# fema-ffrd/gpras

Hardware: AMD Instinct MI355X
Metric: gp_fits_per_sec (higher is better)
Workload: dtype f64; 1 GPU; BASELINE configs[1] as the many-independent-cells workload: exact GP N=4096 d=8 RBF, fit F1 = kernel build + blocked fp64-MFMA Cholesky + alpha + LML, per cell; cells = y columns of one training set with per-cell hyperparameters (the reference's per-mode models); n_train=4096, d=8, kernel=RBF, collective=none (one process), launcher=single process

## Files before the change

gpras_amd/_lib.py:

```python

from __future__ import annotations

import ctypes as C
from pathlib import Path

import numpy as np

import os

LIB_PATH = Path(os.environ["GPRX_LIBRARY"]) if os.environ.get("GPRX_LIBRARY") else Path(__file__).resolve().parent / "libgprx.so"

GPRX_OK, GPRX_EINVAL, GPRX_ENOTPD, GPRX_EHIP, GPRX_ENOMEM, GPRX_ESTATE, GPRX_ERCCL = range(7)
UNIQUE_ID_BYTES = 128
TRAIN_VARIANCE, TRAIN_LENGTHSCALE, TRAIN_NOISE, TRAIN_Z = 1, 2, 4, 8
GEMM_C_LOWER, GEMM_A_LOWER, GEMM_A_UPPER, GEMM_B_LOWER, GEMM_B_UPPER = 1, 2, 4, 8, 16

DISTANCE_FORMS = {"difference": 0, "expanded": 1}
KERNEL_IDS = {"RBF": 0, "Matern12": 1, "Matern32": 2, "Matern52": 3, "Exponential": 4}


class GprxLibraryError(RuntimeError):
    """libgprx.so is missing or unusable."""


# ... 78 lines not shown
    "gprx_ps_destroy": (C.c_int, [_vp]),
    "gprx_ps_last_error": (C.c_char_p, [_vp]),
    "gprx_ps_set_weights": (C.c_int, [_vp, _vp]),
    "gprx_ps_fit_centerline": (C.c_int, [_vp, _vp, _vp, _vp, _vp, _vp, _i64, _vp]),
    "gprx_ps_timings": (C.c_int, [_vp, _dp]),
    "gprx_ps_rating": (C.c_int, [_vp, _vp, _vp, _i64, _vp, _vp]),
    "gprx_ps_set_boundaries": (C.c_int, [_vp, _vp, _vp, _i64]),
    "gprx_ps_centerline": (C.c_int, [_vp, _vp]),
    "gprx_ps_gather": (C.c_int, [_vp, _vp, _i64, _vp]),
    "gprx_ps_surface": (C.c_int, [_vp, _vp, _vp]),
    "gprx_ps_surface_dev": (C.c_int, [_vp, _i64, _i64, _vp, _i64, _vp, _i64]),
    "gprx_ps_synchronize": (C.c_int, [_vp]),
    "gprx_pca_slab_rows": (C.c_int, [_vp, C.POINTER(_i64)]),
    "gprx_metrics": (C.c_int, [C.c_int, _vp, _vp, _vp, _i64, _i64, C.c_int, C.c_double, _vp, _vp, _vp, C.POINTER(C.c_uint64)]),
    "gprx_metrics_dev": (C.c_int, [C.c_int, _vp, _vp, _vp, _i64, _i64, C.c_int, C.c_double, _vp, _vp, _vp, C.POINTER(C.c_uint64)]),
    "gprx_kmeans_pp": (C.c_int, [C.c_int, _vp, _i64, C.c_int, _vp, C.c_int, C.c_int, _i64, _vp, _vp]),
    "gprx_kmeans_lloyd": (C.c_int, [C.c_int, _vp, _i64, C.c_int, _vp, C.c_int, C.c_double, C.c_int, _vp, _ip, _ip]),
    "gprx_gather_rows": (C.c_int, [C.c_int, _vp, _i64, _i64, _vp, _vp]),
    "gprx_kmat": (C.c_int, [C.c_int, C.c_int, _vp, _i64, _vp, _i64, C.c_int, _vp, C.c_double, C.c_double, _vp, _i64, _i64, _i64, C.c_int]),
    "gprx_gemm": (C.c_int, [C.c_int, C.c_int, C.c_int, _i64, _i64, _i64, C.c_double, _vp, _i64, _vp, _i64, C.c_double, _vp, _i64, C.c_int, C.c_int]),
    "gprx_potrf": (C.c_int, [C.c_int, _vp, _i64, _i64, _i64, _vp, _ip]),
    "gprx_set_tuning": (C.c_int, [C.c_char_p, C.c_int]),
    "gprx_set_handle_tuning": (C.c_int, [_vp, C.c_char_p, C.c_int]),
    "gprx_mfma_f64_peak": (C.c_int, [C.c_int, _dp]),
    "gprx_exp_probe": (C.c_int, [C.c_int, C.c_int, _vp, _i64, _vp]),
}

_lib = None


def load():
    global _lib
    if _lib is not None:
        return _lib
    if not LIB_PATH.exists():
        raise GprxLibraryError(
            f"{LIB_PATH} not found: build it with `python -c 'import __graft_entry__ as g; g.build()'` "
            "(hipcc --offload-arch=gfx950).  gpras_amd has no CPU fallback."
        )
    try:
        lib = C.CDLL(str(LIB_PATH))
    except OSError as exc:
        raise GprxLibraryError(f"cannot load {LIB_PATH}: {exc}") from exc
    for name, (res, args) in PROTOTYPES.items():
        try:
            fn = getattr(lib, name)
# ... 70 lines not shown
```

gpras_amd/csrc/gemm_f64.h:

```cpp
#pragma once
#include <cstdlib>

#include "gprx_common.h"

namespace gprx {

struct GemmArgs {
  const double* A;
  const double* B;
  double* C;
  int64_t lda, ldb, ldc;
  int M, N, K;
  double alpha, beta;
  int flags;
  int tiles_n;
  int tiles_m;
  int nwg;
  int64_t strideA, strideB, strideC;
  int ksplit;
  int64_t slab;
  int inner = 0;
  int64_t cellA = 0, cellB = 0, cellC = 0;
  const double* a_sub = nullptr;
  const double* a_mul = nullptr;
  const double* a_elev = nullptr;
  const double* alpha_tab = nullptr;
  int alpha_stride = 0;
  int persist_slots = 0;
  double* rowsq = nullptr;
  int64_t rowsq_ld = 0;
  int cell_xcd = 0;
};

#ifndef GPRX_GEMM_PFC_DEFAULT
#define GPRX_GEMM_PFC_DEFAULT 1
#endif
#ifndef GPRX_GEMM_DMA_DEFAULT
#define GPRX_GEMM_DMA_DEFAULT 1
#endif
constexpr int GEMM_BK = 16;
constexpr int GEMM_LDK = GEMM_BK;
__device__ __forceinline__ int kc_swz(int row) { return (int)((0xa7a09f5366f7ull >> (3 * (row & 15))) & 7ull); }

template <int BMN>
struct McStride {
  static constexpr int value = BMN + 4;
};

template <int ROWS>
__device__ __forceinline__ void load_kc(d2 (&r)[ROWS / 32], const double* __restrict__ base, int64_t ld, int row0, int nrows_valid,
                                        int k0, int tid) {
#pragma unroll
  for (int i = 0; i < ROWS / 32; ++i) {
    const int q = tid + 256 * i;
    const int row = q >> 3, cc = q & 7;
    if (row0 + row < nrows_valid)
      r[i] = *reinterpret_cast<const d2*>(base + (int64_t)(row0 + row) * ld + k0 + cc * 2);
    else
      r[i] = d2{0.0, 0.0};
  }
}
template <int ROWS>
__device__ __forceinline__ void store_kc(double* s, const d2 (&r)[ROWS / 32], int tid) {
// ... 22 lines not shown
  }
}
template <int COLS>
__device__ __forceinline__ void store_mc(double* s, const d2 (&r)[COLS / 32], int tid) {
#pragma unroll
  for (int i = 0; i < COLS / 32; ++i) {
    const int q = tid + 256 * i;
    const int krow = q / (COLS / 2), cc = q % (COLS / 2);
    *reinterpret_cast<d2*>(s + krow * McStride<COLS>::value + cc * 2) = r[i];
  }
}

__device__ __forceinline__ void glds16(const double* src, double* lds_wave_base) {
  __builtin_amdgcn_global_load_lds((const __attribute__((address_space(1))) void*)src, (__attribute__((address_space(3))) void*)lds_wave_base, 16, 0, 0);
}

template <int TA, int TB, int BM, int BN>
struct GemmSmem {
  static constexpr int A_ELEMS = TA ? GEMM_BK * McStride<BM>::value : BM * GEMM_LDK;
  static constexpr int B_ELEMS = TB ? BN * GEMM_LDK : GEMM_BK * McStride<BN>::value;
  static constexpr int doubles = 2 * (A_ELEMS + B_ELEMS);
};

template <int TA, int TB, int BM, int BN, int PF, int AXF, int DMA>
__device__ __forceinline__ void gemm_tile(GemmArgs p, const int bx_in, const int by_in, const int bz, double* __restrict__ smem) {
  int bx = bx_in, by = by_in;
  if (p.cell_xcd) {
    const int L = bx_in + p.nwg * by_in, slot = L >> 3;
    const int cq = slot / p.nwg;
    by = (L & 7) + 8 * cq;
    bx = slot - cq * p.nwg;
  }
  static_assert(!DMA || (AXF == 0 && (TA == 0 || BM == 64) && (TB == 1 || BN == 64)),
                "the LDS-DMA staging exists for k-contiguous operands and for m/n-contiguous operands of 64-wide tiles");
  constexpr int TM = BM / 32, TN = BN / 32;
  constexpr int A_ELEMS = GemmSmem<TA, TB, BM, BN>::A_ELEMS;
  constexpr int B_ELEMS = GemmSmem<TA, TB, BM, BN>::B_ELEMS;

  const int tid = threadIdx.x;
  const int lane = tid & 63;
  const int wave = tid >> 6;
  const int wm = wave >> 1, wn = wave & 1;
  const int g = lane >> 4, r = lane & 15;

  {
    int entry = by;
    if (p.inner > 0) {
      const int cell = entry / p.inner;
      entry -= cell * p.inner;
      p.A += (int64_t)cell * p.cellA;
      p.B += (int64_t)cell * p.cellB;
      p.C += (int64_t)cell * p.cellC;
      if (p.alpha_tab) p.alpha = p.alpha_tab[(int64_t)cell * p.alpha_stride];
    }
    p.A += (int64_t)entry * p.strideA;
    p.B += (int64_t)entry * p.strideB;
    p.C += (int64_t)entry * p.strideC;
  }
  int bid = bx;
  if (!p.cell_xcd && !(p.flags & (GEMM_A_LOWER | GEMM_A_UPPER | GEMM_B_LOWER | GEMM_B_UPPER))) {
    const int q = p.nwg >> 3, rr = p.nwg & 7, xcd = bid & 7, k = bid >> 3;
    bid = (xcd < rr ? xcd * (q + 1) : rr * (q + 1) + (xcd - rr) * q) + k;
  }
  int ti, tj;
  if (p.flags & GEMM_C_LOWER) {
#ifndef GPRX_BAND
#define GPRX_BAND 4
#endif
    constexpr int R = GPRX_BAND;
    const int tn = p.tiles_n;
    const int tri = tn * (tn + 1) / 2;
    if (bid < tri) {
      int b = (int)((sqrtf((float)(R + 1) * (R + 1) / 4.0f - (float)(R + 1) * R / 2.0f + (float)R * R / 4.0f + 2.0f * (float)bid) -
                     (float)(R + 1) / 2.0f + (float)R / 2.0f) / (float)R);
      if (b < 0) b = 0;
      auto S = [](int bb) { return R * R * bb * (bb - 1) / 2 + bb * R * (R + 1) / 2; };
      while (S(b + 1) <= bid) ++b;
      while (S(b) > bid) --b;
      int u = bid - S(b);
      const int r0 = R * b;
      const int h = (tn - r0 < R) ? tn - r0 : R;
      if (u < h * r0) {
        tj = u / h;
        ti = r0 + u % h;
      } else {
        u -= h * r0;
        int c = 0;
        while (u >= h - c) {
          u -= h - c;
          ++c;
        }
        tj = r0 + c;
        ti = r0 + c + u;
      }
    } else {
      const int rest = bid - tri;
      const int b2 = rest / (R * tn);
      const int u = rest - b2 * R * tn;
      const int left = p.tiles_m - tn - R * b2;
      const int h = left < R ? left : R;
      tj = u / h;
      ti = tn + R * b2 + u % h;
    }
  } else {
    const int tri = p.flags & (GEMM_A_LOWER | GEMM_A_UPPER | GEMM_B_LOWER | GEMM_B_UPPER);
    if (tri == GEMM_B_UPPER || tri == GEMM_B_LOWER) {
      const int cj = bid / p.tiles_m;
      ti = bid % p.tiles_m;
      tj = (tri == GEMM_B_UPPER) ? p.tiles_n - 1 - cj : cj;
    } else if (tri == GEMM_A_LOWER || tri == GEMM_A_UPPER) {
      const int ri = bid / p.tiles_n;
      tj = bid % p.tiles_n;
      ti = (tri == GEMM_A_LOWER) ? p.tiles_m - 1 - ri : ri;
    } else {
      ti = bid / p.tiles_n;
      tj = bid % p.tiles_n;
      if (tri & (GEMM_B_LOWER | GEMM_B_UPPER)) tj = (tj + ti) % p.tiles_n;
    }
  }
  const int m0 = ti * BM, n0 = tj * BN;

  int kbeg = 0, kend = p.K;
  if (p.flags & GEMM_A_LOWER) kend = min(kend, m0 + BM);
  if (p.flags & GEMM_A_UPPER) kbeg = max(kbeg, m0);
  if (p.flags & GEMM_B_LOWER) kbeg = max(kbeg, n0);
  if (p.flags & GEMM_B_UPPER) kend = min(kend, n0 + BN);
// ... 241 lines not shown
#pragma unroll
        for (int q = 0; q < 4; ++q) {
          const int row = m0 + wm * (BM / 2) + a * 16 + g + 4 * q;
          cold[b][q] = (row < p.M && col < p.N) ? p.C[(int64_t)row * p.ldc + col] : 0.0;
        }
      }
    }
#pragma unroll
    for (int b = 0; b < TN; ++b) {
      const int col = n0 + wn * (BN / 2) + b * 16 + r;
#pragma unroll
      for (int q = 0; q < 4; ++q) {
        const int row = m0 + wm * (BM / 2) + a * 16 + g + 4 * q;
        if (row < p.M && col < p.N) {
          double v = alpha * acc[a][b][q];
          if (beta != 0.0) v = __builtin_fma(beta, cold[b][q], v);
          p.C[(int64_t)row * p.ldc + col] = v;
        }
      }
    }
  }
}

template <int TA, int TB, int BM, int BN, int PF = 0, int AXF = 0, int DMA = 0>
__global__ __launch_bounds__(256, (BM * BN >= 128 * 128) ? 2 : (((PF && !DMA) || AXF) ? 3 : 4)) void gemm_f64_kernel(GemmArgs p) {
  __shared__ __attribute__((aligned(16))) double smem[GemmSmem<TA, TB, BM, BN>::doubles];
  gemm_tile<TA, TB, BM, BN, PF, AXF, DMA>(p, (int)blockIdx.x, (int)blockIdx.y, (int)blockIdx.z, smem);
}

template <int BM, int BN, int PF>
__global__ __launch_bounds__(256, (BM * BN >= 128 * 128) ? 2 : 4) void gemm_f64_nt_dma_persistent_kernel(GemmArgs p, int batch) {
  __shared__ __attribute__((aligned(16))) double smem[GemmSmem<0, 1, BM, BN>::doubles];
  const int total = p.nwg * batch;
  for (int t = (int)blockIdx.x; t < total; t += (int)gridDim.x) {
    const int by = t / p.nwg;
    gemm_tile<0, 1, BM, BN, PF, 0, 1>(p, t - by * p.nwg, by, 0, smem);
  }
}

template <int TA, int TB, int BM, int BN>
inline hipError_t launch_gemm_t(hipStream_t st, GemmArgs p, int batch, int nsplit = 1) {
  p.tiles_m = (p.M + BM - 1) / BM;
  p.tiles_n = (p.N + BN - 1) / BN;
  if (p.tiles_m == 0 || p.tiles_n == 0) return hipSuccess;
  if (p.flags & GEMM_C_LOWER) {
    if (p.tiles_n > p.tiles_m) p.tiles_n = p.tiles_m;
    p.nwg = p.tiles_n * (p.tiles_n + 1) / 2 + (p.tiles_m - p.tiles_n) * p.tiles_n;
  } else {
    p.nwg = p.tiles_m * p.tiles_n;
  }
  {
    static const int cell_xcd = getenv("GPRX_CELL_XCD") ? atoi(getenv("GPRX_CELL_XCD")) : 1;
    p.cell_xcd = (cell_xcd && p.inner == 0 && nsplit == 1 && batch >= 8 && batch % 8 == 0 && p.persist_slots == 0 &&
                  !(p.flags & (GEMM_A_LOWER | GEMM_A_UPPER | GEMM_B_LOWER | GEMM_B_UPPER))) ? 1 : 0;
  }
  if constexpr (TA == 0 && TB == 1) {
    static const int dma = getenv("GPRX_GEMM_DMA") ? atoi(getenv("GPRX_GEMM_DMA")) : GPRX_GEMM_DMA_DEFAULT;
    static const int pfc = getenv("GPRX_GEMM_PFC") ? atoi(getenv("GPRX_GEMM_PFC")) : GPRX_GEMM_PFC_DEFAULT;
    if (dma && p.M % BM == 0 && p.N % BN == 0 && p.K % GEMM_BK == 0 && p.lda % 2 == 0 && p.ldb % 2 == 0) {
      const bool prefetch_c = BM * BN <= 64 * 64 && p.beta != 0.0 && nsplit == 1 && (pfc >= 2 || (pfc == 1 && p.K <= 128));
      if (p.persist_slots > 0 && nsplit == 1 && !prefetch_c) {
        static const int n_cu = [] {
          int dev = 0, cus = 256;
          hipGetDevice(&dev);
          hipDeviceGetAttribute(&cus, hipDeviceAttributeMultiprocessorCount, dev);
          return cus > 0 ? cus : 256;
        }();
        int grid = p.persist_slots * n_cu;
        grid -= grid % 8;
        if (grid > 0 && (int64_t)p.nwg * batch > grid) {
          hipLaunchKernelGGL((gemm_f64_nt_dma_persistent_kernel<BM, BN, 0>), dim3(grid), dim3(256), 0, st, p, batch);
          return hipGetLastError();
        }
      }
      static const int pad_env = getenv("GPRX_GEMM_PAD_LDS") ? atoi(getenv("GPRX_GEMM_PAD_LDS")) : -1;
      const unsigned pad = (batch == 1 && BM * BN <= 64 * 64) ? (unsigned)(pad_env >= 0 ? pad_env : 0) : 0u;
      if (prefetch_c)
        hipLaunchKernelGGL((gemm_f64_kernel<0, 1, (BM > 64 ? 64 : BM), (BN > 64 ? 64 : BN), 1, 0, 1>), dim3(p.nwg, batch, nsplit), dim3(256), pad, st, p);
      else
        hipLaunchKernelGGL((gemm_f64_kernel<0, 1, BM, BN, 0, 0, 1>), dim3(p.nwg, batch, nsplit), dim3(256), pad, st, p);
      return hipGetLastError();
    }
  }
  if constexpr (TA == 0 && TB == 0 && BM == 64 && BN == 64) {
    static const int dma_nn = getenv("GPRX_GEMM_DMA_NN") ? atoi(getenv("GPRX_GEMM_DMA_NN")) : 1;
    if (dma_nn && p.M % BM == 0 && p.N % BN == 0 && p.K % GEMM_BK == 0 && p.lda % 2 == 0 && p.ldb % 2 == 0 && nsplit == 1 &&
        (reinterpret_cast<uintptr_t>(p.A) & 15) == 0 && (reinterpret_cast<uintptr_t>(p.B) & 15) == 0 && p.strideA % 2 == 0 && p.strideB % 2 == 0 &&
        p.cellA % 2 == 0 && p.cellB % 2 == 0) {
      hipLaunchKernelGGL((gemm_f64_kernel<0, 0, 64, 64, 0, 0, 1>), dim3(p.nwg, batch, nsplit), dim3(256), 0, st, p);
      return hipGetLastError();
// ... 102 lines not shown
    for (int b = 0; b < 2; ++b) {
      const int col = n0 + wn * 32 + b * 16 + r;
#pragma unroll
      for (int q = 0; q < 4; ++q) {
        const int row = m0 + wm * 32 + a * 16 + g + 4 * q;
        if (row < M && col < N) C[(int64_t)row * ldc + col] = acc[a][b][q];
      }
    }
}

inline hipError_t launch_syrk_k64(hipStream_t st, int M, int N, const double* A, int64_t lda, double* C, int64_t ldc, int batch = 1,
                                  int64_t cs = 0) {
  const int tm = (M + 63) / 64;
  int tn = (N + 63) / 64;
  if (tm == 0 || tn == 0) return hipSuccess;
  if (tn > tm) tn = tm;
  const int nwg = tn * (tn + 1) / 2 + (tm - tn) * tn;
  hipLaunchKernelGGL(syrk_k64_kernel, dim3(nwg, batch), dim3(256), 0, st, A, A, C, lda, ldc, M, N, tn, cs);
  return hipGetLastError();
}
inline hipError_t launch_gemm(hipStream_t st, int ta, int tb, int M, int N, int K, double alpha, const double* A, int64_t lda, const double* B,
                              int64_t ldb, double beta, double* C, int64_t ldc, int flags, int tile, int batch, int64_t strideA, int64_t strideB,
                              int64_t strideC, int cells, int64_t cellA, int64_t cellB, int64_t cellC, const double* alpha_tab, int alpha_stride,
                              int persist_slots, double* rowsq, int64_t rowsq_ld);
inline hipError_t launch_update_k64(hipStream_t st, int M, int N, const double* A, int64_t lda, double* C, int64_t ldc, int batch, int64_t cs) {
  static const int via_gemm = getenv("GPRX_K64_GEMM") ? atoi(getenv("GPRX_K64_GEMM")) : 1;
  if (!via_gemm) return launch_syrk_k64(st, M, N, A, lda, C, ldc, batch, cs);
  return launch_gemm(st, 0, 1, M, N, 64, -1.0, A, lda, A, lda, 1.0, C, ldc, GEMM_C_LOWER, 64, batch, cs, cs, cs, 1, 0, 0, 0, nullptr, 0, 0, nullptr, 0);
}

inline hipError_t launch_gemm(hipStream_t st, int ta, int tb, int M, int N, int K, double alpha, const double* A, int64_t lda,
                              const double* B, int64_t ldb, double beta, double* C, int64_t ldc, int flags, int tile = 0, int batch = 1,
                              int64_t strideA = 0, int64_t strideB = 0, int64_t strideC = 0, int cells = 1, int64_t cellA = 0,
                              int64_t cellB = 0, int64_t cellC = 0, const double* alpha_tab = nullptr, int alpha_stride = 0, int persist_slots = 0,
                              double* rowsq = nullptr, int64_t rowsq_ld = 0) {
  GemmArgs p{A, B, C, lda, ldb, ldc, M, N, K, alpha, beta, flags, 0, 0, 0, strideA, strideB, strideC, 0, 0};
  p.persist_slots = persist_slots;
  p.rowsq = rowsq;
  p.rowsq_ld = rowsq_ld;
  if (M <= 0 || N <= 0 || batch <= 0 || cells <= 0) return hipSuccess;
  if (cells > 1 || alpha_tab) {
    p.inner = batch;
    p.cellA = cellA;
    p.cellB = cellB;
    p.cellC = cellC;
    p.alpha_tab = alpha_tab;
    p.alpha_stride = alpha_stride;
    batch *= cells;
  }
  static const int force_tile = getenv("GPRX_FORCE_TILE") ? atoi(getenv("GPRX_FORCE_TILE")) : 0;
  if (force_tile) tile = force_tile;
  if (tile == 0) {
    const int64_t t128 = (int64_t)batch * ((M + 127) / 128) * ((N + 127) / 128) / ((flags & GEMM_C_LOWER) ? 2 : 1);
    tile = (t128 >= 1024) ? 128 : 64;
  }
#define GPRX_GEMM_CASE(TA_, TB_)                                                  \
  if (ta == TA_ && tb == TB_) {                                                   \
    if (tile == 128) return launch_gemm_t<TA_, TB_, 128, 128>(st, p, batch);      \
    return launch_gemm_t<TA_, TB_, 64, 64>(st, p, batch);                         \
  }
// ... 72 lines not shown
```

gpras_amd/csrc/gprx.hip:

```cpp
#include "../../include/gprx.h"

#include <hip/hip_runtime.h>

#include <algorithm>
#include <chrono>
#include <cmath>
#include <cstdio>
#include <cstdlib>
#include <cstring>
#include <limits>
#include <map>
#include <mutex>
#include <string>
#include <thread>
#include <vector>

#include "comm.h"
#include "gemm_f64.h"
#include "gprx_common.h"
#include "grad.h"
#include "hms.h"
#include "kmat.h"
#include "kmeans.h"
#include "metrics.h"
// ... 4252 lines not shown
#ifdef GPRX_PANEL_STAMPS
int gprx_panel_stamps(unsigned long long* out64) {
  hipMemcpyFromSymbol(out64, HIP_SYMBOL(gprx::g_panel_stamps), sizeof(unsigned long long) * 64);
  return 0;
}
#endif

namespace {
bool apply_tuning(PotrfTuning& t, int& predict_path, int& fused, const std::string& k, int value) {
  if (k == "panel_width" && (value == 0 || value == 64 || value == 128)) t.panel_width = value;
  else if (k == "outer_block" && value >= 0 && value % 128 == 0) t.outer_block = value;
  else if (k == "update_tile" && (value == 0 || value == 64 || value == 128)) t.update_tile = value;
  else if (k == "no_lookahead") t.no_lookahead = value != 0;
  else if (k == "panel_rows" && (value == 0 || value == 128 || value == 256)) t.panel_rows = value;
  else if (k == "panel_occ" && (value == 0 || value == 2 || value == 3)) t.panel_occ = value;
  else if (k == "inblock" && (value == 0 || value == 1)) t.inblock = value;
  else if (k == "split_panel" && value >= -1 && value <= 1) t.split_panel = value;
  else if (k == "dag" && value >= -1 && value <= 1) t.dag = value;
  else if (k == "rhs_vector" && value >= -1 && value <= 1) t.rhs_vector = value;
  else if (k == "rows_inv" && value >= -1 && value <= 1) t.rows_inv = value;
  else if (k == "rows_inv_rt" && value >= 0 && value <= 2) t.rows_inv_rt = value;
  else if (k == "rows_inv_lone" && value >= 0 && value <= 1) t.rows_inv_lone = value;
  else if (k == "cell_kernel" && value >= -1 && value <= 1) t.cell_kernel = value;
  else if (k == "split_updates" && value >= 0 && value <= 1) t.split_updates = value;
  else if (k == "poison_workspace" && value >= 0 && value <= 1) t.poison_workspace = value;
  else if (k == "predict_path" && value >= 0 && value <= 2) predict_path = value;
  else if (k == "sgpr_fused" && value >= 0 && value <= 1) fused = value;
  else if (k == "wait_handover_us" && value >= 0) wait_handover_us() = value;
  else if (k == "sgpr_groups_from" && value >= 0) sf_groups_from() = value;
  else return false;
  return true;
}
}

int gprx_set_tuning(const char* key, int value) {
  if (!key) return fail(nullptr, GPRX_EINVAL, "null key");
  if (!apply_tuning(potrf_tuning(), predict_path_tuning(), sgpr_fused_tuning(), key, value)) return fail(nullptr, GPRX_EINVAL, "unknown tuning key or bad value");
  return GPRX_OK;
}

int gprx_set_handle_tuning(gprx_handle h, const char* key, int value) {
  if (!h || !key) return fail(h, GPRX_EINVAL, "null argument");
  const int fused_before = h->sgpr_fused;
  if (!apply_tuning(h->tune, h->predict_path, h->sgpr_fused, key, value)) return fail(h, GPRX_EINVAL, "unknown tuning key or bad value");
  if (hipSetDevice(h->device) == hipSuccess && hipStreamSynchronize(h->stream) == hipSuccess) drop_graphs(h);
  if (h->sgpr_fused != fused_before) {
    h->sarena_slots = 0;
    h->factorized = h->sparse_view ? false : h->factorized;
    h->sparse_view = false;
  }
  return GPRX_OK;
}

int gprx_mfma_f64_peak(int device, double* tflops) {
  if (!tflops) return fail(nullptr, GPRX_EINVAL, "null argument");
  HIPCHK(nullptr, hipSetDevice(device));
  double* out = nullptr;
  HIPCHK(nullptr, hipMalloc((void**)&out, 64));
  hipEvent_t e0, e1;
  hipEventCreate(&e0);
  hipEventCreate(&e1);
  const int iters = 20000, blocks = 256 * 4;
  hipStream_t us = util_stream();
  hipLaunchKernelGGL(mfma_f64_peak_kernel, dim3(blocks), dim3(256), 0, us, out, 100);
  hipEventRecord(e0, us);
  hipLaunchKernelGGL(mfma_f64_peak_kernel, dim3(blocks), dim3(256), 0, us, out, iters);
  hipEventRecord(e1, us);
  hipError_t e = hipStreamSynchronize(us);
  float ms = 0.f;
  hipEventElapsedTime(&ms, e0, e1);
  hipEventDestroy(e0);
  hipEventDestroy(e1);
  hipFree(out);
  HIPCHK(nullptr, e);
  const double flops = (double)blocks * 4  * iters * 4  * 2048.0;
// ... 6 lines not shown
```

gpras_amd/csrc/potrf.h:

```cpp
#pragma once
#include <cstdlib>
#include <utility>
#include <vector>

#include "chain64.h"
#include "gemm_f64.h"
#include "gprx_common.h"

namespace gprx {

#ifdef GPRX_PANEL_ACC
__device__ unsigned long long g_panel_acc[8];
#define PACC_DECL unsigned long long pacc_prev_ = 0;
#define PACC(i)                                                                                                       \
  {                                                                                                                   \
    if ((i) == 5) __builtin_amdgcn_s_waitcnt(0);                                                                      \
    const unsigned long long t_ = __builtin_amdgcn_s_memtime();                                                       \
    if (threadIdx.x == 0 && blockIdx.x == 0 && blockIdx.y == 0 && gridDim.x > 2) {                                    \
      if ((i) > 0) atomicAdd(&g_panel_acc[i], t_ - pacc_prev_);                                                       \
      else atomicAdd(&g_panel_acc[0], 1ull);                                                                          \
    }                                                                                                                 \
    pacc_prev_ = t_;                                                                                                  \
  }
#else
// ... 1066 lines not shown
  }
  ~PotrfProfile() {
    for (auto e : pool) hipEventDestroy(e);
  }
};

struct PotrfTuning {
  int panel_width = 0;
  int outer_block = 0;
  int update_tile = 0;
  int no_lookahead = 0;
  int panel_rows = 0;
  int panel_occ = 0;
  int inblock = 0;
  int split_panel = 0;
  int poison_workspace = 0;
  int split_updates = 0;
  int cell_kernel = 0;
  int rhs_vector = 0;
  int rows_inv = 0;
  int rows_inv_rt = 0;
  int rows_inv_lone = 0;
  int dag = 0;
};
inline PotrfTuning& potrf_tuning() {
  static PotrfTuning t = [] {
    PotrfTuning v;
    if (const char* e = getenv("GPRX_OUTER_BLOCK")) v.outer_block = atoi(e);
    if (const char* e = getenv("GPRX_UPDATE_TILE")) v.update_tile = atoi(e);
    if (const char* e = getenv("GPRX_PANEL_ROWS")) v.panel_rows = atoi(e);
    if (const char* e = getenv("GPRX_PANEL_WIDTH")) v.panel_width = atoi(e);
    if (const char* e = getenv("GPRX_PANEL_OCC")) v.panel_occ = atoi(e);
    if (const char* e = getenv("GPRX_INBLOCK")) v.inblock = atoi(e);
    if (const char* e = getenv("GPRX_SPLIT_PANEL")) v.split_panel = atoi(e);
    if (const char* e = getenv("GPRX_DAG")) v.dag = atoi(e);
    if (const char* e = getenv("GPRX_RHS_VECTOR")) v.rhs_vector = atoi(e);
    if (const char* e = getenv("GPRX_ROWS_INV")) v.rows_inv = atoi(e);
    if (const char* e = getenv("GPRX_ROWS_INV_RT")) v.rows_inv_rt = atoi(e);
    if (const char* e = getenv("GPRX_ROWS_INV_LONE")) v.rows_inv_lone = atoi(e);
    if (const char* e = getenv("GPRX_SPLIT_UPDATES")) v.split_updates = atoi(e);
    if (const char* e = getenv("GPRX_CELL_KERNEL")) v.cell_kernel = atoi(e);
    return v;
  }();
  return t;
}

struct PotrfStreams {
  hipStream_t aux = nullptr;
  hipStream_t side = nullptr;
  std::vector<hipEvent_t> pool;
  size_t used = 0;
  hipEvent_t block_done = nullptr, tail_done = nullptr;
  hipEvent_t next_event() {
    if (used == pool.size()) {
      hipEvent_t e = nullptr;
      if (hipEventCreateWithFlags(&e, hipEventDisableTiming) != hipSuccess) return nullptr;
      pool.push_back(e);
    }
    return pool[used++];
  }
  hipError_t init() {
    hipError_t e = hipStreamCreateWithFlags(&aux, hipStreamNonBlocking);
    if (e != hipSuccess) return e;
    if ((e = hipStreamCreateWithFlags(&side, hipStreamNonBlocking)) != hipSuccess) return e;
// ... 22 lines not shown

inline hipError_t potrf_lower(hipStream_t st, double* A, int64_t lda, int np, int extra, double* inv_diag, int* info,
                              double* diag_stage, PotrfProfile* prof = nullptr, PotrfStreams* ps = nullptr, int batch = 1, int64_t cs = 0,
                              int info_stride = 0, const PotrfTuning* tune_in = nullptr, int col_base = 0, hipEvent_t first_block_evt = nullptr,
                              double* yvec = nullptr) {
  const double* prev_stage = nullptr;
  double* prev_dst = nullptr;
  int prev_pw = 0;
  auto mark_gemm = [&](hipStream_t s, int ncols_lower, int rows_rect, int ncols, int k, bool strip = false) {
    if (!prof) return;
    const double elems = 0.5 * (double)ncols_lower * (ncols_lower + 1) + (double)rows_rect * ncols;
    (strip ? prof->strip_marks : prof->gemm_marks).push_back({prof->used, 2.0 * k * elems * batch});
    hipEventRecord(prof->next(), s);
  };
  auto mark_end = [&](hipStream_t s) {
    if (prof) hipEventRecord(prof->next(), s);
  };
  const int total_rows = np + extra;
  const PotrfTuning& tune = tune_in ? *tune_in : potrf_tuning();
  if (tune.no_lookahead) ps = nullptr;
  const int ob = tune.outer_block ? tune.outer_block : (np > 4096 ? 512 : 1024);
  const int pwidth = tune.panel_width ? tune.panel_width : NB;
  const int bulk_tile = tune.update_tile ? tune.update_tile : 64;
  bool tail_pending = false;
  static const int tail_slots = getenv("GPRX_TAIL_SLOTS") ? atoi(getenv("GPRX_TAIL_SLOTS")) : 0;
  hipError_t err = hipSuccess;
  const bool rows_inv = tune.rows_inv > 0;
  const int rows_inv_rt = tune.rows_inv_rt == 2 ? 2 : 1;
  const bool split_panel = tune.split_panel ? tune.split_panel > 0 : (batch >= 24 || (rows_inv && tune.rows_inv_lone > 0));
  static const bool fuse_ok = [] {
    const char* a = getenv("GPRX_K64_GEMM");
    const char* b = getenv("GPRX_GEMM_DMA");
    const char* c = getenv("GPRX_FUSE_K64");
    return !(a && atoi(a) == 0) && !(b && atoi(b) == 0) && !(c && atoi(c) == 0);
  }();
  struct PendingCols {
    int begin, end;
    hipEvent_t ev;
  };
  std::vector<PendingCols> pending;
  const bool split_ok = ps && ps->side && batch == 1 && !prof && tune.split_updates > 0 && tune.inblock != 1;
  if (split_ok) ps->used = 0;
  auto main_wait = [&](int a, int b) {
    for (size_t q = 0; q < pending.size();) {
      if (pending[q].begin < b && pending[q].end > a) {
        hipStreamWaitEvent(st, pending[q].ev, 0);
// ... 72 lines not shown
      const int own = PanelGeom<2>::kOwnRows;
      const int nchunks = (rows_below + own - 1) / own;
      if (tune.panel_occ == 3)
        hipLaunchKernelGGL((potrf_panel_kernel<2, 3>), dim3(nchunks + 1, batch), dim3(256), 0, st, Acc, lda, rows_below, nchunks, invd, info,
                           col_base + c, stage_out, prev_stage, prev_dst, prev_pw, cs, info_stride);
      else if (fuse)
        hipLaunchKernelGGL((potrf_panel_kernel<2, 2, true>), dim3(nchunks + 1, batch), dim3(256), 0, st, Acc, lda, rows_below, nchunks, invd, info,
                           col_base + c, stage_out, prev_stage, prev_dst, prev_pw, cs, info_stride);
      else
        hipLaunchKernelGGL((potrf_panel_kernel<2, 2>), dim3(nchunks + 1, batch), dim3(256), 0, st, Acc, lda, rows_below, nchunks, invd, info,
                           col_base + c, stage_out, prev_stage, prev_dst, prev_pw, cs, info_stride);
    }
    prev_stage = stage_out;
    prev_dst = Acc;
    prev_pw = pw;
    if (prof) hipEventRecord(prof->next(), st);
  };
  auto update_on = [&](hipStream_t s_, int c0, int k, int c1, int n, int tile) {
    const int rows = total_rows - c1;
    const double* L21 = A + (int64_t)c1 * lda + c0;
    double* A22 = A + (int64_t)c1 * lda + c1;
    mark_gemm(s_, n, rows - n, n, k, k <= 128);
    hipError_t e = (k == NB) ? launch_update_k64(s_, rows, n, L21, lda, A22, lda, batch, cs)
                             : launch_gemm(s_, 0, 1, rows, n, k, -1.0, L21, lda, L21, lda, 1.0, A22, lda, GEMM_C_LOWER, tile, batch, cs, cs, cs);
    mark_end(s_);
    if (e != hipSuccess && err == hipSuccess) err = e;
  };
  auto split_update = [&](int c0, int k, int c1, int n, int tile, hipEvent_t side_wait) {
    if (!split_ok || n <= NB || k < 256) {
      main_wait(c1, c1 + n);
      if (side_wait) hipStreamWaitEvent(st, side_wait, 0);
      update_on(st, c0, k, c1, n, tile);
      return;
    }
    hipEvent_t ready = ps->next_event();
    hipEventRecord(ready, st);
    hipStreamWaitEvent(ps->side, ready, 0);
    if (side_wait) hipStreamWaitEvent(ps->side, side_wait, 0);
    for (int start = NB; start < n;) {
      const int wdt = n - start < start ? n - start : start;
      update_on(ps->side, c0, k, c1 + start, wdt, tile);
      hipEvent_t done = ps->next_event();
      hipEventRecord(done, ps->side);
      pending.push_back({c1 + start, c1 + start + wdt, done});
      start += wdt;
    }
    main_wait(c1, c1 + NB);
// ... 26 lines not shown
        if (strip > 0) inblock_update(c, NB, c + NB, strip);
      }
    } else {
      factor_range(factor_range, C, w);
    }
    if (err != hipSuccess) return err;
    if (C == 0 && first_block_evt) hipEventRecord(first_block_evt, st);
    const int R = C + w;
    if (R >= np) break;
    const int wn = (np - R < ob) ? np - R : ob;
    const double* Lpan = A + (int64_t)R * lda + C;
    split_update(C, w, R, wn, batch > 1 ? bulk_tile : 64, (ps && tail_pending) ? ps->tail_done : nullptr);
    if (err != hipSuccess) return err;
    if (ps) hipEventRecord(ps->block_done, st);
    const int R2 = R + wn;
    if (R2 < np) {
      hipStream_t ts = ps ? ps->aux : st;
      if (ps) hipStreamWaitEvent(ts, ps->block_done, 0);
      const int rows = total_rows - R2, cols = np - R2;
      const double* Lrow = A + (int64_t)R2 * lda + C;
      mark_gemm(ts, cols, rows - cols, cols, w);
      const int persist = (ps && batch == 1) ? tail_slots : 0;
      hipError_t e = launch_gemm(ts, 0, 1, rows, cols, w, -1.0, Lrow, lda, Lrow, lda, 1.0, A + (int64_t)R2 * lda + R2, lda, GEMM_C_LOWER,
                                   bulk_tile, batch, cs, cs, cs, 1, 0, 0, 0, nullptr, 0, persist);
      mark_end(ts);
      if (e != hipSuccess) return e;
      if (ps) {
        hipEventRecord(ps->tail_done, ts);
        tail_pending = true;
      }
    }
  }
  main_wait(0, 1 << 30);
  if (prev_stage) hipLaunchKernelGGL(copy_block_kernel, dim3(batch), dim3(256), 0, st, prev_stage, prev_dst, lda, prev_pw, cs);
  if (ps && tail_pending) hipStreamWaitEvent(st, ps->tail_done, 0);
  return hipGetLastError();
}

}
```

include/gprx.h:

```cpp
#ifndef GPRX_H
#define GPRX_H

#include <stdint.h>

#ifdef __cplusplus
extern "C" {
#endif

#define GPRX_VERSION 100

#define GPRX_OK 0
#define GPRX_EINVAL 1
#define GPRX_ENOTPD 2
#define GPRX_EHIP 3
#define GPRX_ENOMEM 4
#define GPRX_ESTATE 5
#define GPRX_ERCCL 6

#define GPRX_KERNEL_RBF 0
#define GPRX_KERNEL_MATERN12 1
#define GPRX_KERNEL_MATERN32 2
#define GPRX_KERNEL_MATERN52 3
#define GPRX_KERNEL_EXPONENTIAL 4

// ... 140 lines not shown
int gprx_ps_rating(gprx_ps_handle h, const double* us_q, const double* ds_q, int64_t T, double* us_wse, double* ds_wse);
int gprx_ps_set_boundaries(gprx_ps_handle h, const double* us_wse, const double* ds_wse, int64_t T);
int gprx_ps_centerline(gprx_ps_handle h, double* out);
int gprx_ps_gather(gprx_ps_handle h, const double* centerline, int64_t rows, double* out);
int gprx_ps_surface(gprx_ps_handle h, const double* fluvial, double* out);
int gprx_ps_surface_dev(gprx_ps_handle h, int64_t t0, int64_t rows, const double* fluvial_dev, int64_t ldf, double* out_dev, int64_t ldo);
int gprx_ps_synchronize(gprx_ps_handle h);
int gprx_pca_slab_rows(gprx_pca_handle p, int64_t* rows);

int gprx_metrics(int device, const double* x, const double* y, const double* conf, int64_t rows, int64_t cells, int t_tol, double v_tol,
                 double* row_sums, double* cell_sums, int* cell_arg, unsigned long long* matches);
int gprx_metrics_dev(int device, const double* x_dev, const double* y_dev, const double* conf_dev, int64_t rows, int64_t cells, int t_tol,
                     double v_tol, double* row_sums_dev, double* cell_sums_dev, int* cell_arg_dev, unsigned long long* matches);

int gprx_kmeans_pp(int device, const double* x, int64_t n, int d, const double* xsq, int m, int trials, int64_t first_id, const double* uniforms,
                   int64_t* indices_out);
int gprx_kmeans_lloyd(int device, const double* x, int64_t n, int d, double* centers, int m, double tol, int max_iter, int32_t* labels,
                      int* n_iter, int* empty);

int gprx_gather_rows(int device, const double* field_dev, int64_t rows, int64_t cells, const int64_t* idx, double* out);

int gprx_set_tuning(const char* key, int value);
int gprx_set_handle_tuning(gprx_handle h, const char* key, int value);

int gprx_exp_probe(int device, int which, const double* x, int64_t n, double* out);

int gprx_mfma_f64_peak(int device, double* tflops);

#ifdef __cplusplus
}
#endif
#endif
```

Measured before the change: 2314 fits/s.

## Add persistent grid-stride NT GEMM kernel with cross-tile DMA prefetch for batched updates

Adds a persistent variant of the 64x64 LDS-DMA NT GEMM. A fixed grid of about 5 blocks per CU loops over all tiles of a batched trailing update and prefetches the next tile's first K slab while finishing the current one. It is used by default for Cholesky trailing updates when the batch is large enough (at least two rounds of the grid) and K>=256. The aim is to cut block launch and tail overhead and to hide each tile's initial load latency. In exchange it gives up hardware block scheduling and may lose occupancy or load balance on triangular (lower-band) workloads. It also adds a launch counter and a tuning knob.

```diff
diff --git a/gpras_amd/_lib.py b/gpras_amd/_lib.py
--- a/gpras_amd/_lib.py
+++ b/gpras_amd/_lib.py
@@ -124,6 +124,7 @@
     "gprx_potrf": (C.c_int, [C.c_int, _vp, _i64, _i64, _i64, _vp, _ip]),
     "gprx_set_tuning": (C.c_int, [C.c_char_p, C.c_int]),
     "gprx_set_handle_tuning": (C.c_int, [_vp, C.c_char_p, C.c_int]),
+    "gprx_persistent_gemm_launches": (C.c_longlong, []),
     "gprx_mfma_f64_peak": (C.c_int, [C.c_int, _dp]),
     "gprx_exp_probe": (C.c_int, [C.c_int, C.c_int, _vp, _i64, _vp]),
 }
diff --git a/gpras_amd/csrc/gemm_f64.h b/gpras_amd/csrc/gemm_f64.h
--- a/gpras_amd/csrc/gemm_f64.h
+++ b/gpras_amd/csrc/gemm_f64.h
@@ -1,4 +1,5 @@
 #pragma once
+#include <atomic>
 #include <cstdlib>
 
 #include "gprx_common.h"
@@ -30,7 +31,13 @@
   double* rowsq = nullptr;
   int64_t rowsq_ld = 0;
   int cell_xcd = 0;
+  int persist = 0;
+  int persist_total = 0;
 };
+inline std::atomic<long long>& gemm_persist_launches() {
+  static std::atomic<long long> n{0};
+  return n;
+}
 
 #ifndef GPRX_GEMM_PFC_DEFAULT
 #define GPRX_GEMM_PFC_DEFAULT 1
@@ -39,6 +46,9 @@
 #define GPRX_GEMM_DMA_DEFAULT 1
 #endif
 constexpr int GEMM_BK = 16;
+#ifndef GEMM_PERSIST_MIN_ROUNDS
+#define GEMM_PERSIST_MIN_ROUNDS 2
+#endif
 constexpr int GEMM_LDK = GEMM_BK;
 __device__ __forceinline__ int kc_swz(int row) { return (int)((0xa7a09f5366f7ull >> (3 * (row & 15))) & 7ull); }
 
@@ -107,6 +117,46 @@
   static constexpr int doubles = 2 * (A_ELEMS + B_ELEMS);
 };
 
+#ifndef GPRX_BAND
+#define GPRX_BAND 4
+#endif
+__device__ __forceinline__ void lower_band_tile(int bid, int tn, int tiles_m, int& ti, int& tj) {
+  constexpr int R = GPRX_BAND;
+  const int tri = tn * (tn + 1) / 2;
+  if (bid < tri) {
+    int b = (int)((sqrtf((float)(R + 1) * (R + 1) / 4.0f - (float)(R + 1) * R / 2.0f + (float)R * R / 4.0f + 2.0f * (float)bid) -
+                   (float)(R + 1) / 2.0f + (float)R / 2.0f) / (float)R);
+    if (b < 0) b = 0;
+    auto S = [](int bb) { return R * R * bb * (bb - 1) / 2 + bb * R * (R + 1) / 2; };
+    while (S(b + 1) <= bid) ++b;
+    while (S(b) > bid) --b;
+    int u = bid - S(b);
+    const int r0 = R * b;
+    const int h = (tn - r0 < R) ? tn - r0 : R;
+    if (u < h * r0) {
+      tj = u / h;
+      ti = r0 + u % h;
+    } else {
+      u -= h * r0;
+      int c = 0;
+      while (u >= h - c) {
+        u -= h - c;
+        ++c;
+      }
+      tj = r0 + c;
+      ti = r0 + c + u;
+    }
+  } else {
+    const int rest = bid - tri;
+    const int b2 = rest / (R * tn);
+    const int u = rest - b2 * R * tn;
+    const int left = tiles_m - tn - R * b2;
+    const int h = left < R ? left : R;
+    tj = u / h;
+    ti = tn + R * b2 + u % h;
+  }
+}
+
 template <int TA, int TB, int BM, int BN, int PF, int AXF, int DMA>
 __device__ __forceinline__ void gemm_tile(GemmArgs p, const int bx_in, const int by_in, const int bz, double* __restrict__ smem) {
   int bx = bx_in, by = by_in;
@@ -149,44 +199,7 @@
   }
   int ti, tj;
   if (p.flags & GEMM_C_LOWER) {
-#ifndef GPRX_BAND
-#define GPRX_BAND 4
-#endif
-    constexpr int R = GPRX_BAND;
-    const int tn = p.tiles_n;
-    const int tri = tn * (tn + 1) / 2;
-    if (bid < tri) {
-      int b = (int)((sqrtf((float)(R + 1) * (R + 1) / 4.0f - (float)(R + 1) * R / 2.0f + (float)R * R / 4.0f + 2.0f * (float)bid) -
-                     (float)(R + 1) / 2.0f + (float)R / 2.0f) / (float)R);
-      if (b < 0) b = 0;
-      auto S = [](int bb) { return R * R * bb * (bb - 1) / 2 + bb * R * (R + 1) / 2; };
-      while (S(b + 1) <= bid) ++b;
-      while (S(b) > bid) --b;
-      int u = bid - S(b);
-      const int r0 = R * b;
-      const int h = (tn - r0 < R) ? tn - r0 : R;
-      if (u < h * r0) {
-        tj = u / h;
-        ti = r0 + u % h;
-      } else {
-        u -= h * r0;
-        int c = 0;
-        while (u >= h - c) {
-          u -= h - c;
-          ++c;
-        }
-        tj = r0 + c;
-        ti = r0 + c + u;
-      }
-    } else {
-      const int rest = bid - tri;
-      const int b2 = rest / (R * tn);
-      const int u = rest - b2 * R * tn;
-      const int left = p.tiles_m - tn - R * b2;
-      const int h = left < R ? left : R;
-      tj = u / h;
-      ti = tn + R * b2 + u % h;
-    }
+    lower_band_tile(bid, p.tiles_n, p.tiles_m, ti, tj);
   } else {
     const int tri = p.flags & (GEMM_A_LOWER | GEMM_A_UPPER | GEMM_B_LOWER | GEMM_B_UPPER);
     if (tri == GEMM_B_UPPER || tri == GEMM_B_LOWER) {
@@ -474,9 +487,160 @@
   }
 }
 
+struct PersistTile {
+  const double* A;
+  const double* B;
+  double* C;
+};
+__device__ __forceinline__ PersistTile persist_decode(const GemmArgs& p, int L) {
+  int by, bid;
+  if (p.cell_xcd) {
+    const int slot = L >> 3, cq = slot / p.nwg;
+    by = (L & 7) + 8 * cq;
+    bid = slot - cq * p.nwg;
+  } else {
+    by = L / p.nwg;
+    bid = L - by * p.nwg;
+    const int q = p.nwg >> 3, rr = p.nwg & 7, xcd = bid & 7, k = bid >> 3;
+    bid = (xcd < rr ? xcd * (q + 1) : rr * (q + 1) + (xcd - rr) * q) + k;
+  }
+  int ti, tj;
+  if (p.flags & GEMM_C_LOWER) {
+    lower_band_tile(bid, p.tiles_n, p.tiles_m, ti, tj);
+  } else {
+    ti = bid / p.tiles_n;
+    tj = bid % p.tiles_n;
+  }
+  by = __builtin_amdgcn_readfirstlane(by);
+  ti = __builtin_amdgcn_readfirstlane(ti);
+  tj = __builtin_amdgcn_readfirstlane(tj);
+  PersistTile t;
+  t.A = p.A + (int64_t)by * p.strideA + (int64_t)ti * 64 * p.lda;
+  t.B = p.B + (int64_t)by * p.strideB + (int64_t)tj * 64 * p.ldb;
+  t.C = p.C + (int64_t)by * p.strideC + (int64_t)ti * 64 * p.ldc + tj * 64;
+  return t;
+}
+
+__device__ __forceinline__ void gemm_nt_dma_persist_tiles(const GemmArgs& p, double* __restrict__ smem) {
+  constexpr int BM = 64, BN = 64, TM = 2, TN = 2;
+  constexpr int A_ELEMS = GemmSmem<0, 1, BM, BN>::A_ELEMS, B_ELEMS = GemmSmem<0, 1, BM, BN>::B_ELEMS;
+  const int total = p.persist_total, stride = (int)gridDim.x;
+  int L = (int)blockIdx.x;
+  if (L >= total) return;
+  const int tid = threadIdx.x, lane = tid & 63, wave = tid >> 6;
+  const int wm = wave >> 1, wn = wave & 1, g = lane >> 4, r = lane & 15;
+  const int wave_u = __builtin_amdgcn_readfirstlane(wave);
+  const int row0 = wave_u * 8 + (lane >> 3);
+  const unsigned offA = 8u * (unsigned)(row0 * (int)p.lda + 2 * ((lane & 7) ^ kc_swz(row0)));
+  const unsigned offB = 8u * (unsigned)(row0 * (int)p.ldb + 2 * ((lane & 7) ^ kc_swz(row0)));
+  const unsigned offC = 8u * (unsigned)((wm * (BM / 2) + g) * (int)p.ldc + wn * (BN / 2) + r);
+  auto at = [](const double* base, unsigned off) {
+    asm volatile("" : "+v"(off));
+    return reinterpret_cast<const double*>(reinterpret_cast<const char*>(base) + off);
+  };
+  auto dma_fill = [&](const PersistTile& t, int k0, int buf) {
+    double* sa = smem + buf * (A_ELEMS + B_ELEMS);
+    double* sb = sa + A_ELEMS;
+#pragma unroll
+    for (int i = 0; i < BM / 32; ++i) glds16(at(t.A + (int64_t)i * 32 * p.lda + k0, offA), sa + (i * 4 + wave_u) * 8 * GEMM_LDK);
+#pragma unroll
+    for (int i = 0; i < BN / 32; ++i) glds16(at(t.B + (int64_t)i * 32 * p.ldb + k0, offB), sb + (i * 4 + wave_u) * 8 * GEMM_LDK);
+  };
+  const int swz = kc_swz(r);
+  d4 acc[TM][TN];
+  auto mfma_stage = [&](int buf) {
+    const double* sa = smem + buf * (A_ELEMS + B_ELEMS);
+    const double* sb = sa + A_ELEMS;
+    double fa[TM][4], fb[TN][4];
+#pragma unroll
+    for (int a = 0; a < TM; ++a) {
+      const int row = wm * (BM / 2) + a * 16 + r;
+      const d2 lo = *reinterpret_cast<const d2*>(sa + row * GEMM_LDK + 2 * ((2 * g) ^ swz));
+      const d2 hi = *reinterpret_cast<const d2*>(sa + row * GEMM_LDK + 2 * ((2 * g + 1) ^ swz));
+      fa[a][0] = lo.x; fa[a][1] = lo.y; fa[a][2] = hi.x; fa[a][3] = hi.y;
+    }
+#pragma unroll
+    for (int b = 0; b < TN; ++b) {
+      const int col = wn * (BN / 2) + b * 16 + r;
+      const d2 lo = *reinterpret_cast<const d2*>(sb + col * GEMM_LDK + 2 * ((2 * g) ^ swz));
+      const d2 hi = *reinterpret_cast<const d2*>(sb + col * GEMM_LDK + 2 * ((2 * g + 1) ^ swz));
+      fb[b][0] = lo.x; fb[b][1] = lo.y; fb[b][2] = hi.x; fb[b][3] = hi.y;
+    }
+#pragma unroll
+    for (int j = 0; j < 4; ++j)
+#pragma unroll
+      for (int a = 0; a < TM; ++a)
+#pragma unroll
+        for (int b = 0; b < TN; ++b) acc[a][b] = __builtin_amdgcn_mfma_f64_16x16x4f64(fa[a][j], fb[b][j], acc[a][b], 0, 0, 0);
+  };
+  auto stage = [&](const PersistTile& t, int k0, int buf) {
+    dma_fill(t, k0 + GEMM_BK, buf ^ 1);
+    mfma_stage(buf);
+    __syncthreads();
+  };
+  const double alpha = p.alpha, beta = p.beta;
+  const int K = p.K;
+  PersistTile cur = persist_decode(p, L);
+  int buf = 0;
+  dma_fill(cur, 0, buf);
+  __syncthreads();
+  for (;;) {
+    const int Ln = L + stride;
+    const bool has_next = Ln < total;
+    const PersistTile nxt = persist_decode(p, has_next ? Ln : L);
+#pragma unroll
+    for (int a = 0; a < TM; ++a)
+#pragma unroll
+      for (int b = 0; b < TN; ++b) acc[a][b] = d4{0.0, 0.0, 0.0, 0.0};
+    int k0 = 0;
+    for (; k0 + 2 * GEMM_BK < K; k0 += 2 * GEMM_BK) {
+      stage(cur, k0, buf);
+      stage(cur, k0 + GEMM_BK, buf ^ 1);
+    }
+    if (k0 + GEMM_BK < K) {
+      stage(cur, k0, buf);
+      buf ^= 1;
+    }
+    if (has_next) dma_fill(nxt, 0, buf ^ 1);
+    mfma_stage(buf);
+    buf ^= 1;
+    asm volatile("" ::: "memory");
+    __builtin_amdgcn_sched_barrier(0);
+    double cold[TM][TN][4] = {};
+    if (beta != 0.0) {
+#pragma unroll
+      for (int a = 0; a < TM; ++a)
+#pragma unroll
+        for (int b = 0; b < TN; ++b)
+#pragma unroll
+          for (int q = 0; q < 4; ++q) cold[a][b][q] = *at(cur.C + (int64_t)(a * 16 + 4 * q) * p.ldc + b * 16, offC);
+    }
+    __syncthreads();
+#pragma unroll
+    for (int a = 0; a < TM; ++a)
+#pragma unroll
+      for (int b = 0; b < TN; ++b)
+#pragma unroll
+        for (int q = 0; q < 4; ++q) {
+          double v = alpha * acc[a][b][q];
+          if (beta != 0.0) v = __builtin_fma(beta, cold[a][b][q], v);
+          *const_cast<double*>(at(cur.C + (int64_t)(a * 16 + 4 * q) * p.ldc + b * 16, offC)) = v;
+        }
+    if (!has_next) break;
+    cur = nxt;
+    L = Ln;
+  }
+}
+
 template <int TA, int TB, int BM, int BN, int PF = 0, int AXF = 0, int DMA = 0>
 __global__ __launch_bounds__(256, (BM * BN >= 128 * 128) ? 2 : (((PF && !DMA) || AXF) ? 3 : 4)) void gemm_f64_kernel(GemmArgs p) {
   __shared__ __attribute__((aligned(16))) double smem[GemmSmem<TA, TB, BM, BN>::doubles];
+  if constexpr (TA == 0 && TB == 1 && BM == 64 && BN == 64 && PF == 0 && AXF == 0 && DMA == 1) {
+    if (p.persist_total > 0) {
+      gemm_nt_dma_persist_tiles(p, smem);
+      return;
+    }
+  }
   gemm_tile<TA, TB, BM, BN, PF, AXF, DMA>(p, (int)blockIdx.x, (int)blockIdx.y, (int)blockIdx.z, smem);
 }
 
@@ -511,13 +675,29 @@
     static const int pfc = getenv("GPRX_GEMM_PFC") ? atoi(getenv("GPRX_GEMM_PFC")) : GPRX_GEMM_PFC_DEFAULT;
     if (dma && p.M % BM == 0 && p.N % BN == 0 && p.K % GEMM_BK == 0 && p.lda % 2 == 0 && p.ldb % 2 == 0) {
       const bool prefetch_c = BM * BN <= 64 * 64 && p.beta != 0.0 && nsplit == 1 && (pfc >= 2 || (pfc == 1 && p.K <= 128));
+      static const int n_cu = [] {
+        int dev = 0, cus = 256;
+        hipGetDevice(&dev);
+        hipDeviceGetAttribute(&cus, hipDeviceAttributeMultiprocessorCount, dev);
+        return cus > 0 ? cus : 256;
+      }();
+      if constexpr (BM == 64 && BN == 64) {
+        constexpr int64_t kLdMax = (int64_t)1 << 22;
+        const int64_t total = (int64_t)p.nwg * batch;
+        int grid = 5 * n_cu;
+        grid -= grid % 8;
+        const bool eligible = p.persist > 0 && p.persist_slots == 0 && nsplit == 1 && !prefetch_c && p.inner == 0 && !p.rowsq && p.ksplit == 0 && p.K >= 256 &&
+                              !(p.flags & (GEMM_A_LOWER | GEMM_A_UPPER | GEMM_B_LOWER | GEMM_B_UPPER)) && p.lda < kLdMax && p.ldb < kLdMax &&
+                              p.ldc < kLdMax && total < ((int64_t)1 << 30) && grid > 0;
+        if (eligible && (p.persist >= 2 || (batch > 1 && total >= (int64_t)GEMM_PERSIST_MIN_ROUNDS * grid))) {
+          if (total < grid) grid = (int)total;
+          p.persist_total = (int)total;
+          gemm_persist_launches().fetch_add(1, std::memory_order_relaxed);
+          hipLaunchKernelGGL((gemm_f64_kernel<0, 1, 64, 64, 0, 0, 1>), dim3(grid), dim3(256), 0, st, p);
+          return hipGetLastError();
+        }
+      }
       if (p.persist_slots > 0 && nsplit == 1 && !prefetch_c) {
-        static const int n_cu = [] {
-          int dev = 0, cus = 256;
-          hipGetDevice(&dev);
-          hipDeviceGetAttribute(&cus, hipDeviceAttributeMultiprocessorCount, dev);
-          return cus > 0 ? cus : 256;
-        }();
         int grid = p.persist_slots * n_cu;
         grid -= grid % 8;
         if (grid > 0 && (int64_t)p.nwg * batch > grid) {
@@ -666,20 +846,21 @@
 inline hipError_t launch_gemm(hipStream_t st, int ta, int tb, int M, int N, int K, double alpha, const double* A, int64_t lda, const double* B,
                               int64_t ldb, double beta, double* C, int64_t ldc, int flags, int tile, int batch, int64_t strideA, int64_t strideB,
                               int64_t strideC, int cells, int64_t cellA, int64_t cellB, int64_t cellC, const double* alpha_tab, int alpha_stride,
-                              int persist_slots, double* rowsq, int64_t rowsq_ld);
+                              int persist_slots, double* rowsq, int64_t rowsq_ld, int persist);
 inline hipError_t launch_update_k64(hipStream_t st, int M, int N, const double* A, int64_t lda, double* C, int64_t ldc, int batch, int64_t cs) {
   static const int via_gemm = getenv("GPRX_K64_GEMM") ? atoi(getenv("GPRX_K64_GEMM")) : 1;
   if (!via_gemm) return launch_syrk_k64(st, M, N, A, lda, C, ldc, batch, cs);
-  return launch_gemm(st, 0, 1, M, N, 64, -1.0, A, lda, A, lda, 1.0, C, ldc, GEMM_C_LOWER, 64, batch, cs, cs, cs, 1, 0, 0, 0, nullptr, 0, 0, nullptr, 0);
+  return launch_gemm(st, 0, 1, M, N, 64, -1.0, A, lda, A, lda, 1.0, C, ldc, GEMM_C_LOWER, 64, batch, cs, cs, cs, 1, 0, 0, 0, nullptr, 0, 0, nullptr, 0, 0);
 }
 
 inline hipError_t launch_gemm(hipStream_t st, int ta, int tb, int M, int N, int K, double alpha, const double* A, int64_t lda,
                               const double* B, int64_t ldb, double beta, double* C, int64_t ldc, int flags, int tile = 0, int batch = 1,
                               int64_t strideA = 0, int64_t strideB = 0, int64_t strideC = 0, int cells = 1, int64_t cellA = 0,
                               int64_t cellB = 0, int64_t cellC = 0, const double* alpha_tab = nullptr, int alpha_stride = 0, int persist_slots = 0,
-                              double* rowsq = nullptr, int64_t rowsq_ld = 0) {
+                              double* rowsq = nullptr, int64_t rowsq_ld = 0, int persist = 0) {
   GemmArgs p{A, B, C, lda, ldb, ldc, M, N, K, alpha, beta, flags, 0, 0, 0, strideA, strideB, strideC, 0, 0};
   p.persist_slots = persist_slots;
+  p.persist = persist;
   p.rowsq = rowsq;
   p.rowsq_ld = rowsq_ld;
   if (M <= 0 || N <= 0 || batch <= 0 || cells <= 0) return hipSuccess;
diff --git a/gpras_amd/csrc/gprx.hip b/gpras_amd/csrc/gprx.hip
--- a/gpras_amd/csrc/gprx.hip
+++ b/gpras_amd/csrc/gprx.hip
@@ -4298,6 +4298,7 @@
   else if (k == "rows_inv_rt" && value >= 0 && value <= 2) t.rows_inv_rt = value;
   else if (k == "rows_inv_lone" && value >= 0 && value <= 1) t.rows_inv_lone = value;
   else if (k == "cell_kernel" && value >= -1 && value <= 1) t.cell_kernel = value;
+  else if (k == "gemm_persist" && value >= -1 && value <= 1) t.gemm_persist = value;
   else if (k == "split_updates" && value >= 0 && value <= 1) t.split_updates = value;
   else if (k == "poison_workspace" && value >= 0 && value <= 1) t.poison_workspace = value;
   else if (k == "predict_path" && value >= 0 && value <= 2) predict_path = value;
@@ -4327,6 +4328,8 @@
   }
   return GPRX_OK;
 }
+
+long long gprx_persistent_gemm_launches(void) { return gemm_persist_launches().load(std::memory_order_relaxed); }
 
 int gprx_mfma_f64_peak(int device, double* tflops) {
   if (!tflops) return fail(nullptr, GPRX_EINVAL, "null argument");
diff --git a/gpras_amd/csrc/potrf.h b/gpras_amd/csrc/potrf.h
--- a/gpras_amd/csrc/potrf.h
+++ b/gpras_amd/csrc/potrf.h
@@ -1112,6 +1112,7 @@
   int rows_inv_rt = 0;
   int rows_inv_lone = 0;
   int dag = 0;
+  int gemm_persist = 0;
 };
 inline PotrfTuning& potrf_tuning() {
   static PotrfTuning t = [] {
@@ -1130,6 +1131,7 @@
     if (const char* e = getenv("GPRX_ROWS_INV_LONE")) v.rows_inv_lone = atoi(e);
     if (const char* e = getenv("GPRX_SPLIT_UPDATES")) v.split_updates = atoi(e);
     if (const char* e = getenv("GPRX_CELL_KERNEL")) v.cell_kernel = atoi(e);
+    if (const char* e = getenv("GPRX_GEMM_PERSIST")) v.gemm_persist = atoi(e);
     return v;
   }();
   return t;
@@ -1198,6 +1200,7 @@
   const int ob = tune.outer_block ? tune.outer_block : (np > 4096 ? 512 : 1024);
   const int pwidth = tune.panel_width ? tune.panel_width : NB;
   const int bulk_tile = tune.update_tile ? tune.update_tile : 64;
+  const int gemm_persist = tune.gemm_persist < 0 ? 0 : tune.gemm_persist + 1;
   bool tail_pending = false;
   static const int tail_slots = getenv("GPRX_TAIL_SLOTS") ? atoi(getenv("GPRX_TAIL_SLOTS")) : 0;
   hipError_t err = hipSuccess;
@@ -1316,7 +1319,8 @@
     double* A22 = A + (int64_t)c1 * lda + c1;
     mark_gemm(s_, n, rows - n, n, k, k <= 128);
     hipError_t e = (k == NB) ? launch_update_k64(s_, rows, n, L21, lda, A22, lda, batch, cs)
-                             : launch_gemm(s_, 0, 1, rows, n, k, -1.0, L21, lda, L21, lda, 1.0, A22, lda, GEMM_C_LOWER, tile, batch, cs, cs, cs);
+                             : launch_gemm(s_, 0, 1, rows, n, k, -1.0, L21, lda, L21, lda, 1.0, A22, lda, GEMM_C_LOWER, tile, batch, cs, cs, cs, 1, 0, 0,
+                                           0, nullptr, 0, 0, nullptr, 0, gemm_persist);
     mark_end(s_);
     if (e != hipSuccess && err == hipSuccess) err = e;
   };
@@ -1389,7 +1393,7 @@
       mark_gemm(ts, cols, rows - cols, cols, w);
       const int persist = (ps && batch == 1) ? tail_slots : 0;
       hipError_t e = launch_gemm(ts, 0, 1, rows, cols, w, -1.0, Lrow, lda, Lrow, lda, 1.0, A + (int64_t)R2 * lda + R2, lda, GEMM_C_LOWER,
-                                   bulk_tile, batch, cs, cs, cs, 1, 0, 0, 0, nullptr, 0, persist);
+                                   bulk_tile, batch, cs, cs, cs, 1, 0, 0, 0, nullptr, 0, persist, nullptr, 0, gemm_persist);
       mark_end(ts);
       if (e != hipSuccess) return e;
       if (ps) {
diff --git a/include/gprx.h b/include/gprx.h
--- a/include/gprx.h
+++ b/include/gprx.h
@@ -186,6 +186,7 @@
 
 int gprx_set_tuning(const char* key, int value);
 int gprx_set_handle_tuning(gprx_handle h, const char* key, int value);
+long long gprx_persistent_gemm_launches(void);
 
 int gprx_exp_probe(int device, int which, const double* x, int64_t n, double* out);
 
```

New measurement: 2043 fits/s. -11.7%, worse.
